# salesforce/LayoutDETR

Hardware: AMD Instinct MI355X
Metric: images/sec G+D fwd-bwd, 256x256 bg x9 elems (higher is better)
Workload: dtype f32

## Files before the change

### layoutdetr_amd/csrc/p3_engine.hip

```cpp
#include <cstdlib>
#include "ldetr_common.hpp"
#include "../../include/ldetr_hip.h"

namespace ldetr {

bool splitk_ws_alloc(long tiles, size_t partial_bytes, float** ws, int** counters);
void note_engine_launch(bool bf16_split_pipe);

typedef unsigned u32x4 __attribute__((ext_vector_type(4)));
typedef __attribute__((address_space(3))) void lds_void;

struct P3Epi {
    float alpha;
    const float* col_scale;
    const float* col_bias;
    const char* res_p3;
    const float* res_f32;
    const char* mask_p3;
    int relu;
    char* out_p3;
    float* out_f32;
};

struct P3NtParams {
// ... 15 lines not shown
    int ngroups;
};

struct P3Group2 {
    const char* A2; const char* B2;
    P3Epi ep2;
};

__device__ __forceinline__ float bf_lo(unsigned w) { return __uint_as_float(w << 16); }
__device__ __forceinline__ float bf_hi(unsigned w) { return __uint_as_float(w & 0xffff0000u); }

__device__ __forceinline__ bool xcd_tile(int b, int mtiles, int ntiles, int xm, int xn, int& tm, int& tn) {
    const int x = b & 7, i = b >> 3, xi = x / xn, xj = x - xi * xn;
    const int mlo = xi * mtiles / xm, mhi = (xi + 1) * mtiles / xm, nlo = xj * ntiles / xn, nhi = (xj + 1) * ntiles / xn;
    const int cn = nhi - nlo;
    if (cn <= 0 || i >= (mhi - mlo) * cn) return false;
    tm = mlo + i / cn; tn = nlo + i - (i / cn) * cn;
    return true;
}

template <int WM, int WN, int TM, int TN, typename RowMap>
__device__ __forceinline__ void p3_wave_epilogue(const P3Epi& ep, float* Cs, const f32x16 (&acc)[TM][TN], int lane, int nbase, int N, RowMap rowmap) {
    constexpr int CP = WN + 4;
    const int cl = lane & 31, kl = lane >> 5;
#pragma unroll
    for (int i = 0; i < TM; i++)
#pragma unroll
        for (int j = 0; j < TN; j++)
#pragma unroll
            for (int r = 0; r < 16; r++)
                Cs[(i * 32 + (r & 3) + 8 * (r >> 2) + 4 * kl) * CP + j * 32 + cl] = acc[i][j][r];
    constexpr int CH = WN / 8;
    constexpr int RPI = 64 / CH;
    const int ch = lane % CH, rl0 = lane / CH;
    const int n = nbase + ch * 8;
    float cs[8], cb[8];
#pragma unroll
    for (int e = 0; e < 8; e++) { cs[e] = ep.alpha; cb[e] = 0.f; }
    if (n < N) {
        if (ep.col_scale) {
            const float4 s0 = *reinterpret_cast<const float4*>(ep.col_scale + n), s1 = *reinterpret_cast<const float4*>(ep.col_scale + n + 4);
            cs[0] *= s0.x; cs[1] *= s0.y; cs[2] *= s0.z; cs[3] *= s0.w; cs[4] *= s1.x; cs[5] *= s1.y; cs[6] *= s1.z; cs[7] *= s1.w;
        }
        if (ep.col_bias) {
            const float4 s0 = *reinterpret_cast<const float4*>(ep.col_bias + n), s1 = *reinterpret_cast<const float4*>(ep.col_bias + n + 4);
            cb[0] = s0.x; cb[1] = s0.y; cb[2] = s0.z; cb[3] = s0.w; cb[4] = s1.x; cb[5] = s1.y; cb[6] = s1.z; cb[7] = s1.w;
        }
    }
#pragma unroll 2
    for (int it = 0; it < WM / RPI; it++) {
        const int rl = it * RPI + rl0;
        const long orow = rowmap(rl);
        if (orow < 0 || n >= N) continue;
        const float4 v0 = *reinterpret_cast<const float4*>(Cs + rl * CP + ch * 8), v1 = *reinterpret_cast<const float4*>(Cs + rl * CP + ch * 8 + 4);
        float v[8] = {v0.x, v0.y, v0.z, v0.w, v1.x, v1.y, v1.z, v1.w};
#pragma unroll
        for (int e = 0; e < 8; e++) v[e] = v[e] * cs[e] + cb[e];
        const long goff = (orow * N + n) * 6;
        if (ep.res_p3) {
            const u32x4 h = *reinterpret_cast<const u32x4*>(ep.res_p3 + goff), md = *reinterpret_cast<const u32x4*>(ep.res_p3 + goff + 16),
                        lo = *reinterpret_cast<const u32x4*>(ep.res_p3 + goff + 32);
#pragma unroll
            for (int e = 0; e < 4; e++) {
                v[2 * e] += bf_lo(h[e]) + (bf_lo(md[e]) + bf_lo(lo[e]));
                v[2 * e + 1] += bf_hi(h[e]) + (bf_hi(md[e]) + bf_hi(lo[e]));
            }
        }
        if (ep.res_f32) {
            const float4 r0 = *reinterpret_cast<const float4*>(ep.res_f32 + orow * N + n), r1 = *reinterpret_cast<const float4*>(ep.res_f32 + orow * N + n + 4);
            v[0] += r0.x; v[1] += r0.y; v[2] += r0.z; v[3] += r0.w; v[4] += r1.x; v[5] += r1.y; v[6] += r1.z; v[7] += r1.w;
        }
        if (ep.relu) {
#pragma unroll
            for (int e = 0; e < 8; e++) v[e] = v[e] < 0.f ? 0.f : v[e];
        }
        if (ep.mask_p3) {
            const u32x4 h = *reinterpret_cast<const u32x4*>(ep.mask_p3 + goff);
#pragma unroll
            for (int e = 0; e < 4; e++) {
                if ((h[e] << 16) - 1u >= 0x7f800000u) v[2 * e] = 0.f;
                if ((h[e] & 0xffff0000u) - 1u >= 0x7f800000u) v[2 * e + 1] = 0.f;
            }
        }
        if (ep.out_f32) {
            *reinterpret_cast<float4*>(ep.out_f32 + orow * N + n) = make_float4(v[0], v[1], v[2], v[3]);
            *reinterpret_cast<float4*>(ep.out_f32 + orow * N + n + 4) = make_float4(v[4], v[5], v[6], v[7]);
        }
        if (ep.out_p3) {
            u32x4 h, md, lo;
#pragma unroll
            for (int e = 0; e < 4; e++) { unsigned a, b, c; split2_bf16_exact(v[2 * e], v[2 * e + 1], a, b, c); h[e] = a; md[e] = b; lo[e] = c; }
            *reinterpret_cast<u32x4*>(ep.out_p3 + goff) = h;
            *reinterpret_cast<u32x4*>(ep.out_p3 + goff + 16) = md;
            *reinterpret_cast<u32x4*>(ep.out_p3 + goff + 32) = lo;
        }
    }
}

template <int TM, int TN, int NT>
__device__ __forceinline__ bool p3_splitk_reduce(f32x16 (&acc)[TM][TN], float* ws, int* ws_count, long tile, int ks, int splitk, int tile_elems, int tid, int* flag) {
    float* slot0 = ws + tile * splitk * (long)tile_elems;
    float* mine = slot0 + (long)ks * tile_elems;
#pragma unroll
    for (int i = 0; i < TM; i++)
#pragma unroll
        for (int j = 0; j < TN; j++)
#pragma unroll
            for (int r = 0; r < 16; r++)
                __hip_atomic_store(mine + ((i * TN + j) * 16 + r) * NT + tid, acc[i][j][r], __ATOMIC_RELAXED, __HIP_MEMORY_SCOPE_AGENT);
    asm volatile("s_waitcnt vmcnt(0)" ::: "memory");
    __syncthreads();
    if (tid == 0) {
        const int old = atomicAdd(ws_count + tile, 1);
        const int last = old == splitk - 1;
        if (last) __hip_atomic_store(ws_count + tile, 0, __ATOMIC_RELAXED, __HIP_MEMORY_SCOPE_AGENT);
        *flag = last;
    }
    __syncthreads();
    const int last = *flag;
    __syncthreads();
    if (!last) return false;
#pragma unroll
    for (int i = 0; i < TM; i++)
#pragma unroll
        for (int j = 0; j < TN; j++)
#pragma unroll
            for (int r = 0; r < 16; r++) acc[i][j][r] = 0.f;
    for (int sl = 0; sl < splitk; sl++) {
        const float* src = slot0 + (long)sl * tile_elems;
#pragma unroll
        for (int i = 0; i < TM; i++)
#pragma unroll
            for (int j = 0; j < TN; j++)
#pragma unroll
                for (int r = 0; r < 16; r++)
                    acc[i][j][r] += __hip_atomic_load(src + ((i * TN + j) * 16 + r) * NT + tid, __ATOMIC_RELAXED, __HIP_MEMORY_SCOPE_AGENT);
    }
    return true;
}

template <int TM, int TN>
__device__ __forceinline__ bool p3_acc_non_finite(const f32x16 (&acc)[TM][TN]) {
    float chk = 0.f;
#pragma unroll
    for (int i = 0; i < TM; i++)
#pragma unroll
        for (int j = 0; j < TN; j++)
#pragma unroll
            for (int r = 0; r < 16; r++) chk = fmaf(acc[i][j][r], 0.f, chk);
    return __builtin_amdgcn_ballot_w64(chk != chk) != 0ull;
}

typedef unsigned int ld128_t __attribute__((__vector_size__(16)));

__device__ __forceinline__ void p3_load_group(const __amdgpu_buffer_rsrc_t rs, unsigned vo, int so, float (&v)[8]) {
    const ld128_t h = __builtin_amdgcn_raw_buffer_load_b128(rs, vo, so, 0), md = __builtin_amdgcn_raw_buffer_load_b128(rs, vo, so + 16, 0),
                  lo = __builtin_amdgcn_raw_buffer_load_b128(rs, vo, so + 32, 0);
#pragma unroll
    for (int e = 0; e < 4; e++) {
        v[2 * e] = bf_lo(h[e]) + (bf_lo(md[e]) + bf_lo(lo[e]));
        v[2 * e + 1] = bf_hi(h[e]) + (bf_hi(md[e]) + bf_hi(lo[e]));
    }
}

__device__ __forceinline__ float p3_load_elem(const __amdgpu_buffer_rsrc_t rs, unsigned row, int c) {
    const unsigned vo = row == 0x80000000u ? row : row + (unsigned)((c >> 3) * 48 + (c & 7) * 2);
    const unsigned h = __builtin_amdgcn_raw_buffer_load_b16(rs, vo, 0, 0), md = __builtin_amdgcn_raw_buffer_load_b16(rs, vo, 16, 0),
                   lo = __builtin_amdgcn_raw_buffer_load_b16(rs, vo, 32, 0);
    return bf_lo(h) + (bf_lo(md) + bf_lo(lo));
}

template <int WM, int WN, int TM, int TN, typename Dot>
__device__ __forceinline__ void p3_cold_tile(f32x16 (&acc)[TM][TN], float* img, int lane, Dot dot) {
    for (int e = lane; e < WM * WN; e += 64) {
        const int row = e / WN, col = e - row * WN;
        const float v = dot(row, col);
        const int i = row >> 5, rr = row & 31, j = col >> 5, cl = col & 31;
        img[((i * TN + j) * 16 + (rr & 3) + 4 * (rr >> 3)) * 64 + ((rr >> 2) & 1) * 32 + cl] = v;
    }
#pragma unroll
    for (int i = 0; i < TM; i++)
#pragma unroll
        for (int j = 0; j < TN; j++)
#pragma unroll
            for (int r = 0; r < 16; r++) acc[i][j][r] = img[((i * TN + j) * 16 + r) * 64 + lane];
}

__device__ __forceinline__ void p3_nt_row(const P3NtParams& p, int m, unsigned& off, unsigned& vm) {
    vm = 0; off = 0;
    if (m >= p.M) return;
    const int hw = p.OH * p.OW;
    const int n = m / hw, rem = m - n * hw, oy = rem / p.OW, ox = rem - oy * p.OW;
    if (p.tap_mode == 0) {
        const int iy = oy * p.stride, ix = ox * p.stride;
        off = (unsigned)(((n * p.H + iy) * p.W + ix) * p.Cin) * 6u;
        if (p.nty * p.ntx == 1) vm = 1u;
        else
            for (int ty = 0; ty < p.nty; ty++)
                for (int tx = 0; tx < p.ntx; tx++) {
                    const int sy = iy - p.pad + p.kh0 + ty, sx = ix - p.pad + p.kw0 + tx;
                    if (sy >= 0 && sy < p.H && sx >= 0 && sx < p.W) vm |= 1u << (ty * p.ntx + tx);
                }
    } else {
        const int dy = oy * p.out_step + p.out_py + p.pad, dx = ox * p.out_step + p.out_px + p.pad;
        const int by = (dy - p.kh0) / p.stride, bx = (dx - p.kw0) / p.stride;
        off = (unsigned)(((n * p.H + by) * p.W + bx) * p.Cin) * 6u;
        for (int ty = 0; ty < p.nty; ty++)
            for (int tx = 0; tx < p.ntx; tx++) {
                const int sy = by - ty, sx = bx - tx;
                if (sy >= 0 && sy < p.H && sx >= 0 && sx < p.W) vm |= 1u << (ty * p.ntx + tx);
            }
    }
}

__device__ __forceinline__ void p3_nt_koff(const P3NtParams& p, int tap, int cc, int& sA, int& sB) {
    const int ty = tap / p.ntx, tx = tap - ty * p.ntx;
    int dpix;
    if (p.tap_mode == 0) dpix = (p.kh0 + ty) * p.W + (p.kw0 + tx);
    else dpix = (p.nty - 1 - ty) * p.W + (p.ntx - 1 - tx);
    sA = dpix * p.Cin * 6 + cc * 192;
    sB = ((p.kh0 + p.tstep * ty) * p.KW + p.kw0 + p.tstep * tx) * p.Cin * 6 + cc * 192;
}

template <int BM, int BN, int NW, bool ONE>
__device__ __forceinline__ void p3_load_tile(const P3NtParams& p, const __amdgpu_buffer_rsrc_t rsA, const __amdgpu_buffer_rsrc_t rsB,
                                             const unsigned* offA, const unsigned* vmA, const unsigned* offB, int& tap, int& cc, int ktpt, bool live,
                                             ld128_t* ra, ld128_t* rb) {
    constexpr int RGA = BM / 16 / NW, RGB = BN / 16 / NW;
    if constexpr (ONE) {
        const int so = cc * 192;
        ++cc;
#pragma unroll
        for (int i = 0; i < RGA; i++) {
            const unsigned vo = live ? offA[i] : 0x80000000u;
#pragma unroll
            for (int j = 0; j < 3; j++) ra[i * 3 + j] = __builtin_amdgcn_raw_buffer_load_b128(rsA, vo, so + j * 64, 0);
        }
#pragma unroll
        for (int i = 0; i < RGB; i++) {
            const unsigned vo = live ? offB[i] : 0x80000000u;
#pragma unroll
            for (int j = 0; j < 3; j++) rb[i * 3 + j] = __builtin_amdgcn_raw_buffer_load_b128(rsB, vo, so + j * 64, 0);
        }
        return;
    }
    int sA, sB;
    p3_nt_koff(p, tap, cc, sA, sB);
#pragma unroll
    for (int i = 0; i < RGA; i++) {
        const unsigned vo = (live && ((vmA[i] >> tap) & 1u)) ? offA[i] : 0x80000000u;
#pragma unroll
        for (int j = 0; j < 3; j++) ra[i * 3 + j] = __builtin_amdgcn_raw_buffer_load_b128(rsA, vo, sA + j * 64, 0);
    }
#pragma unroll
    for (int i = 0; i < RGB; i++) {
        const unsigned vo = live ? offB[i] : 0x80000000u;
#pragma unroll
        for (int j = 0; j < 3; j++) rb[i * 3 + j] = __builtin_amdgcn_raw_buffer_load_b128(rsB, vo, sB + j * 64, 0);
    }
    if (live && ++cc == ktpt) { cc = 0; ++tap; }
}

template <int BM, int BN, int NW>
__device__ __forceinline__ void p3_store_tile(char* sb, int w, int lane, const ld128_t* ra, const ld128_t* rb) {
    constexpr int RGA = BM / 16 / NW, RGB = BN / 16 / NW, A_BYTES = BM * 192;
#pragma unroll
    for (int i = 0; i < RGA; i++)
#pragma unroll
        for (int j = 0; j < 3; j++) *reinterpret_cast<ld128_t*>(sb + ((w * RGA + i) * 3 + j) * 1024 + lane * 16) = ra[i * 3 + j];
#pragma unroll
    for (int i = 0; i < RGB; i++)
#pragma unroll
        for (int j = 0; j < 3; j++) *reinterpret_cast<ld128_t*>(sb + A_BYTES + ((w * RGB + i) * 3 + j) * 1024 + lane * 16) = rb[i * 3 + j];
}

template <int BM, int BN, int NW, int PF, int NST, bool GROUPS, bool ONE = false>
__device__ __forceinline__ void p3_nt_body(P3NtParams p, const P3Group2& g2, const int bx, const int by, const int bz) {
    constexpr int NT = NW * 64;
    constexpr int WGN = (NW == 8 && BN >= 128) ? 4 : 2, WGM = NW / WGN;
    constexpr int WM = BM / WGM, WN = BN / WGN, TM = WM / 32, TN = WN / 32;
    constexpr int A_BYTES = BM * 192, B_BYTES = BN * 192, ST_BYTES = A_BYTES + B_BYTES;
    constexpr int RGA = BM / 16 / NW, RGB = BN / 16 / NW;
    static_assert(TM >= 1 && TN >= 1 && RGA >= 1 && RGB >= 1 && BM % (16 * NW) == 0 && BN % (16 * NW) == 0, "tile / wave-count mismatch");
    extern __shared__ __attribute__((aligned(1024))) char p3_smem[];
    const int tid = threadIdx.x, lane = tid & 63, w = __builtin_amdgcn_readfirstlane(tid >> 6), wm = w / WGN, wn = w % WGN;
    const int cl = lane & 31, kl = lane >> 5;

    int ws_tile0 = 0;
    if (p.nclass > 1) {
        const int sd = p.stride, cls = p.nclass - 1 - bz, py = cls / sd, px = cls - py * sd;
        ws_tile0 = cls * p.mtiles * p.ntiles;
        p.kh0 = (py + p.pad) % sd; p.kw0 = (px + p.pad) % sd;
        p.nty = p.kh0 < p.KH ? (p.KH - p.kh0 + sd - 1) / sd : 0; p.ntx = p.kw0 < p.KW ? (p.KW - p.kw0 + sd - 1) / sd : 0;
        const int ntaps = p.nty * p.ntx;
        if (ntaps == 0) { p.nty = 0; p.ntx = 1; }
        const unsigned shift = (unsigned)(((p.nty > 0 ? p.nty - 1 : 0) * p.W + (p.ntx - 1)) * p.Cin) * 6u;
        p.A -= shift; p.a_bytes += shift;
        p.OH = (p.out_H - py + sd - 1) / sd; p.OW = (p.out_W - px + sd - 1) / sd;
        p.M = p.nimg * p.OH * p.OW; p.out_py = py; p.out_px = px;
        p.nkt = ntaps * p.Cin / 32;
        p.mtiles = (p.M + BM - 1) / BM;
    } else if (GROUPS && p.ngroups > 1 && bz > 0) {
        p.A = g2.A2; p.B = g2.B2; p.ep = g2.ep2;
        ws_tile0 = p.mtiles * p.ntiles;
    }
    int tm, tn;
    if (!xcd_tile(bx, p.mtiles, p.ntiles, p.xm, p.xn, tm, tn)) return;
    const int t = tm * p.ntiles + tn;
    const int m0 = tm * BM, n0 = tn * BN;
    const int ks = by;
    const int per = (p.nkt + p.splitk - 1) / p.splitk;
    const int kt0 = ks * per, kt1 = min(p.nkt, kt0 + per);

    const __amdgpu_buffer_rsrc_t rsA = __builtin_amdgcn_make_buffer_rsrc(const_cast<char*>(p.A), 0, p.a_bytes, 0x00020000);
    const __amdgpu_buffer_rsrc_t rsB = __builtin_amdgcn_make_buffer_rsrc(const_cast<char*>(p.B), 0, p.b_bytes, 0x00020000);

    const int rr = lane >> 2, pq = (lane & 3) ^ ((rr >> 2) & 3);
    const int ktpt = p.Cin >> 5;
    unsigned offA[RGA], vmA[RGA], offB[RGB];
#pragma unroll
    for (int i = 0; i < RGA; i++) {
        unsigned vm, off;
        p3_nt_row(p, m0 + (w * RGA + i) * 16 + rr, off, vm);
        offA[i] = (ONE && vm == 0u) ? 0x80000000u : off + pq * 16; vmA[i] = vm;
    }
#pragma unroll
    for (int i = 0; i < RGB; i++) {
        const int n = n0 + (w * RGB + i) * 16 + rr;
        offB[i] = n < p.N ? (unsigned)n * (unsigned)(p.KH * p.KW * p.Cin) * 6u + pq * 16 : 0x80000000u;
    }

    int tap = ONE ? 0 : kt0 / ktpt, cc = kt0 - tap * ktpt;

    const int frr = cl & 15, frg = cl >> 4;
    unsigned fo[2][3];
#pragma unroll
    for (int s = 0; s < 2; s++)
#pragma unroll
        for (int pl = 0; pl < 3; pl++) {
            const int e = 3 * (2 * s + kl) + pl;
            fo[s][pl] = (unsigned)((frg * 3 + (e >> 2)) * 1024 + frr * 64 + (((e & 3) ^ ((frr >> 2) & 3)) << 4));
        }
    const unsigned foA = (unsigned)(wm * (WM / 16) * 3 * 1024), foB = (unsigned)(A_BYTES + wn * (WN / 16) * 3 * 1024);

    f32x16 acc[TM][TN];
#pragma unroll
    for (int i = 0; i < TM; i++)
#pragma unroll
        for (int j = 0; j < TN; j++)
#pragma unroll
            for (int r = 0; r < 16; r++) acc[i][j][r] = 0.f;

    const int nloc = kt1 - kt0;
    ld128_t ra[PF][RGA * 3], rb[PF][RGB * 3];
#pragma unroll
    for (int d = 0; d < PF; d++) p3_load_tile<BM, BN, NW, ONE>(p, rsA, rsB, offA, vmA, offB, tap, cc, ktpt, d < nloc, ra[d], rb[d]);
    if (nloc > 0) p3_store_tile<BM, BN, NW>(p3_smem, w, lane, ra[0], rb[0]);
    __syncthreads();
    for (int it0 = 0; it0 < nloc; it0 += PF) {
#pragma unroll
        for (int d = 0; d < PF; d++) {
            const int it = it0 + d;
            p3_load_tile<BM, BN, NW, ONE>(p, rsA, rsB, offA, vmA, offB, tap, cc, ktpt, it + PF < nloc, ra[d], rb[d]);
            __builtin_amdgcn_sched_barrier(0);
            if (it < nloc) {
                const char* sb = p3_smem + (it % NST) * ST_BYTES;
#pragma unroll
                for (int s = 0; s < 2; s++) {
                    bf16x8_t a[TM][3], b[TN][3];
#pragma unroll
                    for (int i = 0; i < TM; i++)
#pragma unroll
                        for (int pl = 0; pl < 3; pl++)
                            a[i][pl] = *reinterpret_cast<const bf16x8_t*>(sb + foA + i * (2 * 3 * 1024) + fo[s][pl]);
#pragma unroll
                    for (int j = 0; j < TN; j++)
#pragma unroll
                        for (int pl = 0; pl < 3; pl++)
                            b[j][pl] = *reinterpret_cast<const bf16x8_t*>(sb + foB + j * (2 * 3 * 1024) + fo[s][pl]);
#pragma unroll
                    for (int i = 0; i < TM; i++)
#pragma unroll
                        for (int j = 0; j < TN; j++) {
                            acc[i][j] = __builtin_amdgcn_mfma_f32_32x32x16_bf16(a[i][1], b[j][1], acc[i][j], 0, 0, 0);
                            acc[i][j] = __builtin_amdgcn_mfma_f32_32x32x16_bf16(a[i][0], b[j][2], acc[i][j], 0, 0, 0);
                            acc[i][j] = __builtin_amdgcn_mfma_f32_32x32x16_bf16(a[i][2], b[j][0], acc[i][j], 0, 0, 0);
                            acc[i][j] = __builtin_amdgcn_mfma_f32_32x32x16_bf16(a[i][0], b[j][1], acc[i][j], 0, 0, 0);
                            acc[i][j] = __builtin_amdgcn_mfma_f32_32x32x16_bf16(a[i][1], b[j][0], acc[i][j], 0, 0, 0);
                            acc[i][j] = __builtin_amdgcn_mfma_f32_32x32x16_bf16(a[i][0], b[j][0], acc[i][j], 0, 0, 0);
                        }
                }
                if (NST == 1) __syncthreads();
                if (it + 1 < nloc) p3_store_tile<BM, BN, NW>(p3_smem + ((it + 1) % NST) * ST_BYTES, w, lane, ra[(d + 1) % PF], rb[(d + 1) % PF]);
                __syncthreads();
            }
        }
    }

    constexpr int CP = WN + 4;
    if (p3_acc_non_finite<TM, TN>(acc)) {
        p3_cold_tile<WM, WN, TM, TN>(acc, reinterpret_cast<float*>(p3_smem) + w * (WM * CP), lane, [&](int row, int col) -> float {
            unsigned off, vm;
            p3_nt_row(p, m0 + wm * WM + row, off, vm);
            const int n = n0 + wn * WN + col;
            const unsigned ob = n < p.N ? (unsigned)n * (unsigned)(p.KH * p.KW * p.Cin) * 6u : 0x80000000u;
            float s = 0.f;
            for (int kt = kt0; kt < kt1; kt++) {
                const int tp = kt / ktpt;
                int sA, sB;
                p3_nt_koff(p, tp, kt - tp * ktpt, sA, sB);
                const unsigned vo = ((vm >> tp) & 1u) ? off : 0x80000000u;
                for (int g = 0; g < 4; g++) {
                    float a[8], b[8];
                    p3_load_group(rsA, vo, sA + g * 48, a); p3_load_group(rsB, ob, sB + g * 48, b);
#pragma unroll
                    for (int e = 0; e < 8; e++) s = fmaf(a[e], b[e], s);
                }
            }
            return s;
        });
    }
    if (p.splitk > 1 && !p3_splitk_reduce<TM, TN, NT>(acc, p.ws, p.ws_count, ws_tile0 + t, ks, p.splitk, BM * BN, tid, reinterpret_cast<int*>(p3_smem))) return;
    const int ohw = p.OH * p.OW;
    p3_wave_epilogue<WM, WN, TM, TN>(p.ep, reinterpret_cast<float*>(p3_smem) + w * (WM * CP), acc, lane, n0 + wn * WN, p.N, [&](int rl) -> long {
        const int m = m0 + wm * WM + rl;
        if (m >= p.M) return -1;
        if (p.out_step == 1 && p.out_H == p.OH && p.out_W == p.OW) return m;
        const int nn = m / ohw, rem = m - nn * ohw, oy = rem / p.OW, ox = rem - oy * p.OW;
        return ((long)nn * p.out_H + (oy * p.out_step + p.out_py)) * p.out_W + (ox * p.out_step + p.out_px);
    });
}

template <int BM, int BN, int NW, int PF, int NST, bool ONE = false>
__global__ __launch_bounds__(NW * 64) void p3_nt_kernel(P3NtParams p, P3Group2 g2) { p3_nt_body<BM, BN, NW, PF, NST, true, ONE>(p, g2, blockIdx.x, blockIdx.y, blockIdx.z); }

struct P3C3Params {
    const char* X; const char* Wt;
    unsigned x_bytes, w_bytes;
    int N_img, H, W, Cin, Nout;
    int lgPW, lgPH, NP;
    int HWp, HPIX, NH, NG;
    int ppr, ppi;
    int flip;
    int ncc;
    int splitk; float* ws; int* ws_count;
    int mtiles, ntiles, xm, xn;
    P3Epi ep;
    int ngroups;
};

constexpr int C3_NGMAX = 13, C3_A_BYTES = C3_NGMAX * 3072, C3_B_BYTES = 4 * 3072, C3_LDS = C3_A_BYTES + 3 * C3_B_BYTES;

__device__ __forceinline__ void p3_c3_decode_tile_row(const P3C3Params& p, int tm, int r, int& n, int& y0, int& x0, int& py, int& px) {
    const int lgpp = p.lgPW + p.lgPH;
    const int sp = r >> lgpp, q = r & ((1 << lgpp) - 1);
    py = q >> p.lgPW; px = q & ((1 << p.lgPW) - 1);
    const int pid = tm * p.NP + sp;
    n = pid / p.ppi; const int prem = pid - n * p.ppi;
    const int pr = prem / p.ppr, pc = prem - pr * p.ppr;
    y0 = pr << p.lgPH; x0 = pc << p.lgPW;
}

template <int TAP>
__device__ __forceinline__ void p3_c3_tap(const P3C3Params& p, const __amdgpu_buffer_rsrc_t rsA, const __amdgpu_buffer_rsrc_t rsB, char* smem, int w, int lane,
                                          const unsigned (&offA)[4], unsigned offB, int cc, bool more_cc, bool more_tile,
                                          ld128_t (&ar)[12], ld128_t (&br)[3], const unsigned (&h0)[2], const unsigned (&ce)[2][3], const unsigned (&fo)[2][3],
                                          unsigned foB, f32x16 (&acc)[2][1]) {
    if (more_tile) {
        const int ntap = TAP == 8 ? 0 : TAP + 1, ncc = TAP == 8 ? cc + 1 : cc;
        const int sB = ntap * p.Cin * 6 + ncc * 192;
#pragma unroll
        for (int j = 0; j < 3; j++) br[j] = __builtin_amdgcn_raw_buffer_load_b128(rsB, offB, sB + j * 64, 0);
    }
    if (more_cc) {
#pragma unroll
        for (int q = TAP * 12 / 9; q < (TAP + 1) * 12 / 9; q++)
            ar[q] = __builtin_amdgcn_raw_buffer_load_b128(rsA, offA[q / 3], (cc + 1) * 192 + (q % 3) * 64, 0);
    }
    constexpr int ty = TAP / 3, tx = TAP % 3;
    const int dt = p.flip ? (2 - ty) * p.HWp + (2 - tx) : ty * p.HWp + tx;
    unsigned hb[2], sw[2];
#pragma unroll
    for (int i = 0; i < 2; i++) {
        const unsigned h = h0[i] + dt;
        hb[i] = (h >> 4) * 3072 + ((h & 15) << 6);
        sw[i] = ((h >> 2) & 3) << 4;
    }
    const char* sb = smem + C3_A_BYTES + (TAP % 3) * C3_B_BYTES + foB;
#pragma unroll
    for (int s2 = 0; s2 < 2; s2++) {
        bf16x8_t a[2][3], b[3];
#pragma unroll
        for (int i = 0; i < 2; i++)
#pragma unroll
            for (int pl = 0; pl < 3; pl++) a[i][pl] = *reinterpret_cast<const bf16x8_t*>(smem + hb[i] + (ce[s2][pl] ^ sw[i]));
#pragma unroll
        for (int pl = 0; pl < 3; pl++) b[pl] = *reinterpret_cast<const bf16x8_t*>(sb + fo[s2][pl]);
#pragma unroll
        for (int i = 0; i < 2; i++) {
            acc[i][0] = __builtin_amdgcn_mfma_f32_32x32x16_bf16(a[i][1], b[1], acc[i][0], 0, 0, 0);
            acc[i][0] = __builtin_amdgcn_mfma_f32_32x32x16_bf16(a[i][0], b[2], acc[i][0], 0, 0, 0);
            acc[i][0] = __builtin_amdgcn_mfma_f32_32x32x16_bf16(a[i][2], b[0], acc[i][0], 0, 0, 0);
            acc[i][0] = __builtin_amdgcn_mfma_f32_32x32x16_bf16(a[i][0], b[1], acc[i][0], 0, 0, 0);
            acc[i][0] = __builtin_amdgcn_mfma_f32_32x32x16_bf16(a[i][1], b[0], acc[i][0], 0, 0, 0);
            acc[i][0] = __builtin_amdgcn_mfma_f32_32x32x16_bf16(a[i][0], b[0], acc[i][0], 0, 0, 0);
        }
    }
    if (more_tile) {
        char* dst = smem + C3_A_BYTES + ((TAP + 1) % 3) * C3_B_BYTES + w * 3072 + lane * 16;
#pragma unroll
        for (int j = 0; j < 3; j++) *reinterpret_cast<ld128_t*>(dst + j * 1024) = br[j];
    }
    __syncthreads();
}

template <bool GROUPS>
__device__ __forceinline__ void p3_c3_body(P3C3Params p, const P3Group2& g2, const int bx, const int by, const int bz) {
    constexpr int BM = 128, BN = 64, NT = 256, WM = 64, WN = 32;
    if (GROUPS && p.ngroups > 1 && bz > 0) { p.X = g2.A2; p.Wt = g2.B2; p.ep = g2.ep2; }
    extern __shared__ __attribute__((aligned(1024))) char p3_smem[];
    const int tid = threadIdx.x, lane = tid & 63, w = __builtin_amdgcn_readfirstlane(tid >> 6), wm = w >> 1, wn = w & 1;
    const int cl = lane & 31, kl = lane >> 5;
    int tm, tn;
    if (!xcd_tile(bx, p.mtiles, p.ntiles, p.xm, p.xn, tm, tn)) return;
    const int t = tm * p.ntiles + tn;
    const int n0 = tn * BN;
    const int ks = by;
    const int per = (p.ncc + p.splitk - 1) / p.splitk;
    const int cc0 = ks * per, cc1 = min(p.ncc, cc0 + per);

    const __amdgpu_buffer_rsrc_t rsA = __builtin_amdgcn_make_buffer_rsrc(const_cast<char*>(p.X), 0, p.x_bytes, 0x00020000);
    const __amdgpu_buffer_rsrc_t rsB = __builtin_amdgcn_make_buffer_rsrc(const_cast<char*>(p.Wt), 0, p.w_bytes, 0x00020000);

    const int rr = lane >> 2, pq = (lane & 3) ^ ((rr >> 2) & 3);
    unsigned offA[4], offB;
#pragma unroll
    for (int i = 0; i < 4; i++) {
        const int h = (w + 4 * i) * 16 + rr;
        unsigned off = 0x80000000u;
        if (h < p.NH) {
            const int sp = h / p.HPIX, rem = h - sp * p.HPIX, hy = rem / p.HWp, hx = rem - hy * p.HWp;
            const int pid = tm * p.NP + sp;
            const int n = pid / p.ppi, prem = pid - n * p.ppi, pr = prem / p.ppr, pc = prem - pr * p.ppr;
            const int y = (pr << p.lgPH) + hy - 1, x = (pc << p.lgPW) + hx - 1;
            if (n < p.N_img && y >= 0 && y < p.H && x >= 0 && x < p.W) off = (unsigned)(((n * p.H + y) * p.W + x) * p.Cin) * 6u + pq * 16;
        }
        offA[i] = off;
    }
    {
// ... 337 lines not shown
    p3_c3_body<false>(pc, none, idx % c3_gx, idx / c3_gx, 0);
}

__global__ __launch_bounds__(256) void p3_split_kernel(const float* __restrict__ src, long ld, char* __restrict__ dst, long rows, int C) {
    const int cg = C >> 3;
    const long total = rows * cg;
    for (long u = (long)blockIdx.x * 256 + threadIdx.x; u < total; u += (long)gridDim.x * 256) {
        const long r = u / cg; const int g = (int)(u - r * cg);
        const float4 v0 = *reinterpret_cast<const float4*>(src + r * ld + g * 8), v1 = *reinterpret_cast<const float4*>(src + r * ld + g * 8 + 4);
        const float v[8] = {v0.x, v0.y, v0.z, v0.w, v1.x, v1.y, v1.z, v1.w};
        u32x4 h, md, lo;
#pragma unroll
        for (int e = 0; e < 4; e++) { unsigned a, b, c; split2_bf16_exact(v[2 * e], v[2 * e + 1], a, b, c); h[e] = a; md[e] = b; lo[e] = c; }
        char* d = dst + u * 48;
        *reinterpret_cast<u32x4*>(d) = h; *reinterpret_cast<u32x4*>(d + 16) = md; *reinterpret_cast<u32x4*>(d + 32) = lo;
    }
}

__global__ __launch_bounds__(256) void p3_merge_kernel(const char* __restrict__ src, float* __restrict__ dst, long ld, long rows, int C) {
    const int cg = C >> 3;
    const long total = rows * cg;
    for (long u = (long)blockIdx.x * 256 + threadIdx.x; u < total; u += (long)gridDim.x * 256) {
        const long r = u / cg; const int g = (int)(u - r * cg);
        const char* s = src + u * 48;
        const u32x4 h = *reinterpret_cast<const u32x4*>(s), md = *reinterpret_cast<const u32x4*>(s + 16), lo = *reinterpret_cast<const u32x4*>(s + 32);
        float v[8];
#pragma unroll
        for (int e = 0; e < 4; e++) {
            v[2 * e] = bf_lo(h[e]) + (bf_lo(md[e]) + bf_lo(lo[e]));
            v[2 * e + 1] = bf_hi(h[e]) + (bf_hi(md[e]) + bf_hi(lo[e]));
        }
        *reinterpret_cast<float4*>(dst + r * ld + g * 8) = make_float4(v[0], v[1], v[2], v[3]);
        *reinterpret_cast<float4*>(dst + r * ld + g * 8 + 4) = make_float4(v[4], v[5], v[6], v[7]);
    }
}

__global__ __launch_bounds__(256) void p3_weight_bwd_kernel(const float* __restrict__ w, const float* __restrict__ o_scale, char* __restrict__ dst, int O, int T, int I) {
    const int og = O >> 3;
    const long total = (long)I * T * og;
    for (long u = (long)blockIdx.x * 256 + threadIdx.x; u < total; u += (long)gridDim.x * 256) {
        const int g = (int)(u % og); const long it = u / og; const int tp = (int)(it % T); const int i = (int)(it / T);
        float v[8];
#pragma unroll
        for (int e = 0; e < 8; e++) v[e] = w[((long)(g * 8 + e) * T + tp) * I + i] * (o_scale ? o_scale[g * 8 + e] : 1.f);
        u32x4 h, md, lo;
#pragma unroll
        for (int e = 0; e < 4; e++) { unsigned a, b, c; split2_bf16_exact(v[2 * e], v[2 * e + 1], a, b, c); h[e] = a; md[e] = b; lo[e] = c; }
        char* d = dst + u * 48;
        *reinterpret_cast<u32x4*>(d) = h; *reinterpret_cast<u32x4*>(d + 16) = md; *reinterpret_cast<u32x4*>(d + 32) = lo;
    }
}

__global__ __launch_bounds__(256) void p3_weight_prep_kernel(const long long* __restrict__ table, int nconv) {
    int c = 0;
    while (c + 1 < nconv && (long long)blockIdx.x >= table[(c + 1) * 8 + 7]) ++c;
    const long long* row = table + c * 8;
    const float* w = reinterpret_cast<const float*>(row[0]);
    const float* sc = reinterpret_cast<const float*>(row[1]);
    char* df = reinterpret_cast<char*>(row[2]);
    char* db = reinterpret_cast<char*>(row[3]);
    const int O = (int)row[4], T = (int)row[5], I = (int)row[6];
    const long u = ((long)blockIdx.x - row[7]) * 256 + threadIdx.x;
    const long units = (long)O * T * I / 8;
    if (u >= units) return;
    if (df) {
        const float4 v0 = *reinterpret_cast<const float4*>(w + u * 8), v1 = *reinterpret_cast<const float4*>(w + u * 8 + 4);
        const float v[8] = {v0.x, v0.y, v0.z, v0.w, v1.x, v1.y, v1.z, v1.w};
        u32x4 h, md, lo;
#pragma unroll
        for (int e = 0; e < 4; e++) { unsigned a, b, cc; split2_bf16_exact(v[2 * e], v[2 * e + 1], a, b, cc); h[e] = a; md[e] = b; lo[e] = cc; }
        char* d = df + u * 48;
        *reinterpret_cast<u32x4*>(d) = h; *reinterpret_cast<u32x4*>(d + 16) = md; *reinterpret_cast<u32x4*>(d + 32) = lo;
    }
    if (db) {
        const int i = (int)(u % I); const long r = u / I; const int tp = (int)(r % T); const int g = (int)(r / T);
        float v[8];
#pragma unroll
        for (int e = 0; e < 8; e++) v[e] = w[((long)(g * 8 + e) * T + tp) * I + i] * (sc ? sc[g * 8 + e] : 1.f);
        u32x4 h, md, lo;
#pragma unroll
        for (int e = 0; e < 4; e++) { unsigned a, b, cc; split2_bf16_exact(v[2 * e], v[2 * e + 1], a, b, cc); h[e] = a; md[e] = b; lo[e] = cc; }
        char* d = db + (((long)i * T + tp) * (O / 8) + g) * 48;
        *reinterpret_cast<u32x4*>(d) = h; *reinterpret_cast<u32x4*>(d + 16) = md; *reinterpret_cast<u32x4*>(d + 32) = lo;
    }
}

static void choose_xcd_array(int mtiles, int ntiles, double a_bytes, double b_bytes, int& xm, int& xn, long& grid_x) {
    double best = -1.0; xm = 8; xn = 1;
    for (int n = 1; n <= 8; n *= 2) {
        const int m = 8 / n;
        if ((n > ntiles && n > 1) || (m > mtiles && m > 1)) continue;
        const double cost = a_bytes * n + b_bytes * m;
        if (best < 0 || cost < best) { best = cost; xm = m; xn = n; }
    }
    grid_x = 8L * cdiv(mtiles, xm) * cdiv(ntiles, xn);
}


struct RaisedPerDevice { bool on[64] = {}; };
static bool raise_lds(const void* kern, size_t lds, const char* what, RaisedPerDevice& raised) {
    if (lds <= 64 * 1024) return true;
    int dev = 0;
    if (hipGetDevice(&dev) != hipSuccess || dev < 0 || dev >= 64) dev = -1;
    if (dev >= 0 && raised.on[dev]) return true;
    if (hipFuncSetAttribute(kern, hipFuncAttributeMaxDynamicSharedMemorySize, (int)lds) != hipSuccess) {
        set_error("%s: cannot raise the dynamic LDS limit to %zu bytes", what, lds);
        return false;
    }
    if (dev >= 0) raised.on[dev] = true;
    return true;
}

struct P3LastLaunch { int kind, bm, bn, nw, splitk, xm, xn, ncls, tn_splitk; long grid; };
static thread_local P3LastLaunch t_last = {0, 0, 0, 0, 0, 0, 0, 0, 0, 0};

struct NtGrid { long gx; int sk, ncls; size_t lds; };

template <int BM, int BN, int NW, int NST>
static NtGrid plan_nt(P3NtParams& p, int sk) {
    p.mtiles = cdiv(p.M, BM); p.ntiles = cdiv(p.N, BN);
    NtGrid g; g.ncls = p.nclass > 1 ? p.nclass : (p.ngroups > 1 ? p.ngroups : 1);
    const long nt = (long)p.mtiles * p.ntiles;
    choose_xcd_array(p.mtiles, p.ntiles, (double)p.M * p.Cin * 6.0, (double)p.N * p.KH * p.KW * p.Cin * 6.0, p.xm, p.xn, g.gx);
    if (sk > p.nkt) sk = p.nkt;
    if (sk < 1) sk = 1;
    p.splitk = sk; p.ws = nullptr; p.ws_count = nullptr;
    if (sk > 1 && !splitk_ws_alloc(nt * g.ncls, (size_t)nt * g.ncls * sk * BM * BN * sizeof(float), &p.ws, &p.ws_count)) p.splitk = sk = 1;
    g.sk = sk;
    constexpr int WGN_ = (NW == 8 && BN >= 128) ? 4 : 2, WM_ = BM / (NW / WGN_), WN_ = BN / WGN_;
    constexpr size_t lds_loop = (size_t)NST * (BM + BN) * 192, lds_epi = (size_t)NW * WM_ * (WN_ + 4) * 4;
    g.lds = lds_loop > lds_epi ? lds_loop : lds_epi;
    return g;
}

static long slot_target(double flops, long dflt) {
    static const double small = 1.5 * 1e9;
    return (flops < small && dflt > 256) ? 256 : dflt;
}
static double nt_flops(const P3NtParams& p) { return 2.0 * p.M * p.N * p.nkt * 32.0 * (p.nclass > 1 ? p.nclass : 1); }
static double tn_flops(const P3TnParams& p) { return 2.0 * p.npix * p.Cout * (double)p.Cin * p.KH * p.KW; }

static int nt_splitk(const P3NtParams& p, int bm, int bn, long slots) {
    const long nt = (long)cdiv(p.M, bm) * cdiv(p.N, bn);
    int sk = 1;
    if (nt < slots * 3 / 4) { sk = (int)(slots / nt); if (sk > p.nkt / 4) sk = p.nkt / 4; if (sk > 16) sk = 16; if (sk < 1) sk = 1; }
    return sk;
}

static bool nt_is_plain_gemm(const P3NtParams& p) { return p.KH * p.KW == 1 && p.pad == 0 && p.nclass <= 1 && (p.tap_mode == 0 || p.stride == 1); }

template <int BM, int BN, int NW, int PF, int NST>
static int launch_nt_cfg(P3NtParams& p, const P3Group2& g2, int sk, hipStream_t st) {
    const NtGrid g = plan_nt<BM, BN, NW, NST>(p, sk);
    if constexpr (PF == 1 && NST == 1 && (BM == BN) && (NW == 4 ? BM == 64 : BM == 128)) {
        if (nt_is_plain_gemm(p)) {
            auto kern1 = p3_nt_kernel<BM, BN, NW, PF, NST, true>;
            static RaisedPerDevice raised1;
            if (!raise_lds(reinterpret_cast<const void*>(kern1), g.lds, "p3_nt", raised1)) return LDETR_ERR_LAUNCH;
            hipLaunchKernelGGL(kern1, dim3((unsigned)g.gx, g.sk, g.ncls), NW * 64, g.lds, st, p, g2);
            t_last = {1, BM, BN, NW, g.sk, p.xm, p.xn, g.ncls, 0, g.gx};
            note_engine_launch(true);
            return check_launch("p3_nt");
        }
    }
    auto kern = p3_nt_kernel<BM, BN, NW, PF, NST>;
    static RaisedPerDevice raised;
    if (!raise_lds(reinterpret_cast<const void*>(kern), g.lds, "p3_nt", raised)) return LDETR_ERR_LAUNCH;
    hipLaunchKernelGGL(kern, dim3((unsigned)g.gx, g.sk, g.ncls), NW * 64, g.lds, st, p, g2);
    t_last = {1, BM, BN, NW, g.sk, p.xm, p.xn, g.ncls, 0, g.gx};
    note_engine_launch(true);
    return check_launch("p3_nt");
}

static int launch_nt(P3NtParams& p, const P3Group2& g2, bool forward, hipStream_t st) {
    static const int force_tile = (int)knob("P3_TILE", 0);
    int cfg = 3;
    if (forward && p.nclass <= 1 && ((p.M >= 65536 && p.N >= 128) || (p.M >= 16384 && p.N >= 256 && p.nkt <= 16))) cfg = 1;
    if (force_tile) cfg = force_tile;
    const int bm = cfg == 3 ? 64 : 128, bn = (cfg == 1 || cfg == 4) ? 128 : 64;
    const int sk = nt_splitk(p, bm, bn, slot_target(nt_flops(p), (cfg == 2 || cfg == 3) ? 512 : 256));
    switch (cfg) {
        case 1: return launch_nt_cfg<128, 128, 8, 1, 1>(p, g2, sk, st);
        case 2: return launch_nt_cfg<128, 64, 4, 1, 1>(p, g2, sk, st);
        case 3: return launch_nt_cfg<64, 64, 4, 1, 1>(p, g2, sk, st);
        default: return launch_nt_cfg<128, 128, 4, 1, 1>(p, g2, sk, st);
    }
}

static bool c3_geometry(int N, int H, int W, P3C3Params& p) {
    auto lg = [](int v) { int l = 0; while ((1 << l) < v) ++l; return (1 << l) == v ? l : -1; };
    int PW = W < 16 ? W : 16;
    if (lg(PW) < 0 || W % PW) return false;
    int PH = 128 / PW; if (PH > H) PH = H;
    while (PH > 1 && (H % PH || lg(PH) < 0)) PH >>= 1;
    if (lg(PH) < 0 || H % PH || 128 % (PW * PH)) return false;
    p.lgPW = lg(PW); p.lgPH = lg(PH); p.NP = 128 / (PW * PH);
    p.HWp = PW + 2; p.HPIX = (PH + 2) * (PW + 2); p.NH = p.NP * p.HPIX; p.NG = (p.NH + 15) / 16;
    if (p.NG > C3_NGMAX) return false;
    p.ppr = W / PW; p.ppi = (H / PH) * (W / PW);
    p.N_img = N; p.H = H; p.W = W;
    p.mtiles = (int)(((long)N * p.ppi + p.NP - 1) / p.NP);
    return true;
}

static long plan_c3(P3C3Params& p) {
    p.ntiles = cdiv(p.Nout, 64);
    const long nt = (long)p.mtiles * p.ntiles;
    int sk = 1;
    const long slots = slot_target(2.0 * p.N_img * p.H * p.W * (double)p.Nout * 9.0 * p.Cin, 512);
    if (nt < slots * 3 / 4) { sk = (int)(slots / nt); if (sk > p.ncc / 2) sk = p.ncc / 2; if (sk > 16) sk = 16; if (sk < 1) sk = 1; }
    if (sk > p.ncc) sk = p.ncc;
    p.splitk = sk; p.ws = nullptr; p.ws_count = nullptr;
    const int ng = p.ngroups > 1 ? p.ngroups : 1;
    if (sk > 1 && !splitk_ws_alloc(nt * ng, (size_t)nt * ng * sk * 128 * 64 * sizeof(float), &p.ws, &p.ws_count)) p.splitk = sk = 1;
    long grid_x;
    choose_xcd_array(p.mtiles, p.ntiles, (double)p.N_img * p.H * p.W * p.Cin * 6.0, (double)p.Nout * 9 * p.Cin * 6.0, p.xm, p.xn, grid_x);
    return grid_x;
}

static int launch_c3(P3C3Params& p, const P3Group2& g2, hipStream_t st) {
    const long grid_x = plan_c3(p);
    static RaisedPerDevice raised;
    if (!raise_lds(reinterpret_cast<const void*>(&p3_c3_kernel), C3_LDS, "p3_c3", raised)) return LDETR_ERR_LAUNCH;
    hipLaunchKernelGGL(p3_c3_kernel, dim3((unsigned)grid_x, p.splitk, p.ngroups > 1 ? p.ngroups : 1), 256, C3_LDS, st, p, g2);
    t_last = {2, 128, 64, 4, p.splitk, p.xm, p.xn, p.ngroups > 1 ? p.ngroups : 1, 0, grid_x};
    note_engine_launch(true);
    return check_launch("p3_c3");
}

static void fill_epi(P3Epi& e, const ldetr_p3_epilogue* s) {
    memset(&e, 0, sizeof(e));
    e.alpha = 1.f;
    if (!s) return;
    e.alpha = s->alpha; e.col_scale = s->col_scale; e.col_bias = s->col_bias;
    e.res_p3 = (const char*)s->residual_p3; e.res_f32 = s->residual_f32; e.mask_p3 = (const char*)s->relu_mask_p3; e.relu = s->relu;
}

template <int BM, int BN>
static void plan_tn(P3TnParams& p, int target_blocks) {
    p.mtiles = cdiv(p.Cout, BM); p.ntiles = cdiv(p.Cin, BN);
    const long nt = (long)p.mtiles * p.ntiles * p.KH * p.KW;
    const int nkt = (p.npix + 31) / 32;
    int sk = (int)((target_blocks + nt - 1) / nt);
    if (sk > nkt / 4) sk = nkt / 4;
    if (sk >= 8) sk = (sk + 4) / 8 * 8;
    if (sk < 1) sk = 1;
    p.splitk = sk;
}

template <int BM, int BN, int PF, int NST>
static int launch_tn_cfg(P3TnParams& p, int target_blocks, hipStream_t st) {
    plan_tn<BM, BN>(p, target_blocks);
    const long nt = (long)p.mtiles * p.ntiles * p.KH * p.KW;
    constexpr size_t lds_loop = (size_t)NST * (BM + BN) * 192, lds_cold = (size_t)(BM / 64) * (BN / 64) * 4096 * 4;
    constexpr size_t lds = lds_loop > lds_cold ? lds_loop : lds_cold;
    auto kern = p3_tn_kernel<BM, BN, PF, NST>;
    static RaisedPerDevice raised;
    if (!raise_lds(reinterpret_cast<const void*>(kern), lds, "p3_tn", raised)) return LDETR_ERR_LAUNCH;
    hipLaunchKernelGGL(kern, dim3(p.splitk, (unsigned)nt, 1), 256, lds, st, p);
    t_last = {3, BM, BN, 4, 0, 0, 0, 1, p.splitk, nt};
    note_engine_launch(true);
    return check_launch("p3_tn");
}

static int launch_tn(P3TnParams& p, hipStream_t st) {
    static const int force_tile = (int)knob("P3_WTILE", 0);
    switch (force_tile) {
        case 1: return launch_tn_cfg<128, 128, 1, 1>(p, (int)slot_target(tn_flops(p), 256), st);
        case 2: return launch_tn_cfg<128, 64, 1, 1>(p, (int)slot_target(tn_flops(p), 256), st);
        default: return launch_tn_cfg<64, 64, 1, 1>(p, (int)slot_target(tn_flops(p), 512), st);
    }
}

static int setup_bwd_data(const void* dy, int N, int OH, int OW, int Cout, const void* wb, int Cin, int KH, int KW, int stride, int pad, int IH, int IW,
                          const ldetr_p3_epilogue* ep, void* out_p3, float* out_f32, bool& use_c3, P3C3Params& c, P3NtParams& p) {
    LDETR_CHECK(dy && wb && (out_p3 || out_f32), "p3_conv2d_bwd_data: null operand");
    LDETR_CHECK(Cout % 32 == 0 && Cin % 8 == 0 && KH * KW <= 32 && pad < KH && pad < KW && (stride == 1 || stride == 2),
                "p3_conv2d_bwd_data: unsupported geometry (Cin=%d Cout=%d k=%dx%d stride=%d pad=%d)", Cin, Cout, KH, KW, stride, pad);
    const long dybytes = (long)N * OH * OW * Cout * 6, wbytes = (long)Cin * KH * KW * Cout * 6;
    use_c3 = false;
    if (KH == 3 && KW == 3 && stride == 1 && pad == 1 && OH == IH && OW == IW && dybytes < 0x7fffffffL && wbytes < 0x7fffffffL) {
        memset(&c, 0, sizeof(c));
        if (c3_geometry(N, IH, IW, c)) {
            c.X = (const char*)dy; c.x_bytes = (unsigned)dybytes; c.Wt = (const char*)wb; c.w_bytes = (unsigned)wbytes;
            c.Cin = Cout; c.Nout = Cin; c.flip = 1; c.ncc = Cout / 32;
            fill_epi(c.ep, ep); c.ep.out_p3 = (char*)out_p3; c.ep.out_f32 = out_f32;
            use_c3 = true;
            return LDETR_OK;
        }
    }
    memset(&p, 0, sizeof(p));
    p.B = (const char*)wb; p.b_bytes = (unsigned)wbytes;
    p.N = Cin; p.Cin = Cout; p.KH = KH; p.KW = KW; p.stride = stride; p.pad = pad; p.H = OH; p.W = OW;
    p.out_H = IH; p.out_W = IW; p.out_step = stride; p.tap_mode = 1; p.tstep = stride; p.nimg = N;
    fill_epi(p.ep, ep); p.ep.out_p3 = (char*)out_p3; p.ep.out_f32 = out_f32;
    const long max_shift = ((long)(KH - 1) * OW + (KW - 1)) * Cout * 6;
    LDETR_CHECK(dybytes + max_shift < 0x7fffffffL && wbytes < 0x7fffffffL, "p3_conv2d_bwd_data: tensor too large for 31-bit buffer offsets");
    if (stride == 1) {
        p.kh0 = 0; p.kw0 = 0; p.nty = KH; p.ntx = KW;
        p.A = (const char*)dy - max_shift; p.a_bytes = (unsigned)(dybytes + max_shift);
        p.OH = IH; p.OW = IW; p.M = N * IH * IW; p.nkt = KH * KW * Cout / 32; p.nclass = 1;
    } else {
        p.A = (const char*)dy; p.a_bytes = (unsigned)dybytes;
        p.OH = (IH + stride - 1) / stride; p.OW = (IW + stride - 1) / stride; p.M = N * p.OH * p.OW;
        p.nkt = ((KH + stride - 1) / stride) * ((KW + stride - 1) / stride) * Cout / 32; p.nclass = stride * stride;
        if (p.nkt == 0) p.nkt = 1;
    }
// ... 182 lines not shown
```

Before: 496.3.

## Software-pipeline LDS fragment reads with MFMA in the bf16x3 NT GEMM main loop

Restructures the NT GEMM main loop so LDS fragment reads for the next step are double-buffered in registers and issued while the current step's MFMAs run. The last step's MFMAs are split around the global prefetch, the LDS store and the barrier to hide their latency. It also enables the plain-GEMM kernel variant for two-stage LDS configurations. In exchange it adds register pressure from the doubled fragment buffers, and the new static_assert restricts instantiations to PF==1.

```diff
diff --git a/layoutdetr_amd/csrc/p3_engine.hip b/layoutdetr_amd/csrc/p3_engine.hip
--- a/layoutdetr_amd/csrc/p3_engine.hip
+++ b/layoutdetr_amd/csrc/p3_engine.hip
@@ -191,6 +191,8 @@
 }
 
 typedef unsigned int ld128_t __attribute__((__vector_size__(16)));
+
+constexpr int P3_SPLIT = 2;
 
 __device__ __forceinline__ void p3_load_group(const __amdgpu_buffer_rsrc_t rs, unsigned vo, int so, float (&v)[8]) {
     const ld128_t h = __builtin_amdgcn_raw_buffer_load_b128(rs, vo, so, 0), md = __builtin_amdgcn_raw_buffer_load_b128(rs, vo, so + 16, 0),
@@ -313,6 +315,27 @@
         for (int j = 0; j < 3; j++) *reinterpret_cast<ld128_t*>(sb + A_BYTES + ((w * RGB + i) * 3 + j) * 1024 + lane * 16) = rb[i * 3 + j];
 }
 
+template <int TN>
+__device__ __forceinline__ void p3_read_step(const char* sb, unsigned foA, unsigned foB, const unsigned (&fo)[3], int i, bf16x8_t (&a)[3], bf16x8_t (&b)[TN][3]) {
+#pragma unroll
+    for (int pl = 0; pl < 3; pl++) a[pl] = *reinterpret_cast<const bf16x8_t*>(sb + foA + i * (2 * 3 * 1024) + fo[pl]);
+    if (i == 0) {
+#pragma unroll
+        for (int j = 0; j < TN; j++)
+#pragma unroll
+            for (int pl = 0; pl < 3; pl++) b[j][pl] = *reinterpret_cast<const bf16x8_t*>(sb + foB + j * (2 * 3 * 1024) + fo[pl]);
+    }
+}
+
+template <int TN, int P0, int P1>
+__device__ __forceinline__ void p3_step_mfma(f32x16 (&acc)[TN], const bf16x8_t (&a)[3], const bf16x8_t (&b)[TN][3]) {
+    constexpr int PA[6] = {1, 0, 2, 0, 1, 0}, PB[6] = {1, 2, 0, 1, 0, 0};
+#pragma unroll
+    for (int j = 0; j < TN; j++)
+#pragma unroll
+        for (int q = P0; q < P1; q++) acc[j] = __builtin_amdgcn_mfma_f32_32x32x16_bf16(a[PA[q]], b[j][PB[q]], acc[j], 0, 0, 0);
+}
+
 template <int BM, int BN, int NW, int PF, int NST, bool GROUPS, bool ONE = false>
 __device__ __forceinline__ void p3_nt_body(P3NtParams p, const P3Group2& g2, const int bx, const int by, const int bz) {
     constexpr int NT = NW * 64;
@@ -390,50 +413,38 @@
 #pragma unroll
             for (int r = 0; r < 16; r++) acc[i][j][r] = 0.f;
 
+    static_assert(PF == 1 && (NST == 1 || NST == 2), "one k-tile in registers, one or two LDS stages");
     const int nloc = kt1 - kt0;
-    ld128_t ra[PF][RGA * 3], rb[PF][RGB * 3];
-#pragma unroll
-    for (int d = 0; d < PF; d++) p3_load_tile<BM, BN, NW, ONE>(p, rsA, rsB, offA, vmA, offB, tap, cc, ktpt, d < nloc, ra[d], rb[d]);
-    if (nloc > 0) p3_store_tile<BM, BN, NW>(p3_smem, w, lane, ra[0], rb[0]);
+    ld128_t ra[RGA * 3], rb[RGB * 3];
+    bf16x8_t af[2][3], bfr[2][TN][3];
+    constexpr int NSTEP = 2 * TM;
+    p3_load_tile<BM, BN, NW, ONE>(p, rsA, rsB, offA, vmA, offB, tap, cc, ktpt, 0 < nloc, ra, rb);
+    if (nloc > 0) p3_store_tile<BM, BN, NW>(p3_smem, w, lane, ra, rb);
+    p3_load_tile<BM, BN, NW, ONE>(p, rsA, rsB, offA, vmA, offB, tap, cc, ktpt, 1 < nloc, ra, rb);
     __syncthreads();
-    for (int it0 = 0; it0 < nloc; it0 += PF) {
-#pragma unroll
-        for (int d = 0; d < PF; d++) {
-            const int it = it0 + d;
-            p3_load_tile<BM, BN, NW, ONE>(p, rsA, rsB, offA, vmA, offB, tap, cc, ktpt, it + PF < nloc, ra[d], rb[d]);
+    if (nloc > 0) p3_read_step<TN>(p3_smem, foA, foB, fo[0], 0, af[0], bfr[0]);
+    for (int it = 0; it < nloc; it++) {
+        const char* sb = p3_smem + (NST == 2 ? (it & 1) : 0) * ST_BYTES;
+        char* sn = p3_smem + (NST == 2 ? ((it + 1) & 1) : 0) * ST_BYTES;
+        const bool more = it + 1 < nloc;
+#pragma unroll
+        for (int k = 0; k < NSTEP - 1; k++) {
+            p3_read_step<TN>(sb, foA, foB, fo[(k + 1) / TM], (k + 1) % TM, af[(k + 1) & 1], bfr[(k + 1) / TM]);
             __builtin_amdgcn_sched_barrier(0);
-            if (it < nloc) {
-                const char* sb = p3_smem + (it % NST) * ST_BYTES;
-#pragma unroll
-                for (int s = 0; s < 2; s++) {
-                    bf16x8_t a[TM][3], b[TN][3];
-#pragma unroll
-                    for (int i = 0; i < TM; i++)
-#pragma unroll
-                        for (int pl = 0; pl < 3; pl++)
-                            a[i][pl] = *reinterpret_cast<const bf16x8_t*>(sb + foA + i * (2 * 3 * 1024) + fo[s][pl]);
-#pragma unroll
-                    for (int j = 0; j < TN; j++)
-#pragma unroll
-                        for (int pl = 0; pl < 3; pl++)
-                            b[j][pl] = *reinterpret_cast<const bf16x8_t*>(sb + foB + j * (2 * 3 * 1024) + fo[s][pl]);
-#pragma unroll
-                    for (int i = 0; i < TM; i++)
-#pragma unroll
-                        for (int j = 0; j < TN; j++) {
-                            acc[i][j] = __builtin_amdgcn_mfma_f32_32x32x16_bf16(a[i][1], b[j][1], acc[i][j], 0, 0, 0);
-                            acc[i][j] = __builtin_amdgcn_mfma_f32_32x32x16_bf16(a[i][0], b[j][2], acc[i][j], 0, 0, 0);
-                            acc[i][j] = __builtin_amdgcn_mfma_f32_32x32x16_bf16(a[i][2], b[j][0], acc[i][j], 0, 0, 0);
-                            acc[i][j] = __builtin_amdgcn_mfma_f32_32x32x16_bf16(a[i][0], b[j][1], acc[i][j], 0, 0, 0);
-                            acc[i][j] = __builtin_amdgcn_mfma_f32_32x32x16_bf16(a[i][1], b[j][0], acc[i][j], 0, 0, 0);
-                            acc[i][j] = __builtin_amdgcn_mfma_f32_32x32x16_bf16(a[i][0], b[j][0], acc[i][j], 0, 0, 0);
-                        }
-                }
-                if (NST == 1) __syncthreads();
-                if (it + 1 < nloc) p3_store_tile<BM, BN, NW>(p3_smem + ((it + 1) % NST) * ST_BYTES, w, lane, ra[(d + 1) % PF], rb[(d + 1) % PF]);
-                __syncthreads();
-            }
-        }
+            p3_step_mfma<TN, 0, 6>(acc[k % TM], af[k & 1], bfr[k / TM]);
+            __builtin_amdgcn_sched_barrier(0);
+        }
+        if (NST == 1) __syncthreads();
+        if (more) p3_store_tile<BM, BN, NW>(sn, w, lane, ra, rb);
+        p3_load_tile<BM, BN, NW, ONE>(p, rsA, rsB, offA, vmA, offB, tap, cc, ktpt, it + 2 < nloc, ra, rb);
+        __builtin_amdgcn_sched_barrier(0);
+        p3_step_mfma<TN, 0, P3_SPLIT>(acc[TM - 1], af[1], bfr[1]);
+        __builtin_amdgcn_sched_barrier(0);
+        __syncthreads();
+        if (more) p3_read_step<TN>(sn, foA, foB, fo[0], 0, af[0], bfr[0]);
+        __builtin_amdgcn_sched_barrier(0);
+        p3_step_mfma<TN, P3_SPLIT, 6>(acc[TM - 1], af[1], bfr[1]);
+        __builtin_amdgcn_sched_barrier(0);
     }
 
     constexpr int CP = WN + 4;
@@ -1077,7 +1088,7 @@
 template <int BM, int BN, int NW, int PF, int NST>
 static int launch_nt_cfg(P3NtParams& p, const P3Group2& g2, int sk, hipStream_t st) {
     const NtGrid g = plan_nt<BM, BN, NW, NST>(p, sk);
-    if constexpr (PF == 1 && NST == 1 && (BM == BN) && (NW == 4 ? BM == 64 : BM == 128)) {
+    if constexpr (PF == 1 && (BM == BN) && (NW == 4 ? BM == 64 : BM == 128)) {
         if (nt_is_plain_gemm(p)) {
             auto kern1 = p3_nt_kernel<BM, BN, NW, PF, NST, true>;
             static RaisedPerDevice raised1;
```

Result: no change. 497.4, median of 3 (+0.2%).
